# jason2714/de-i2i-gan

Measured on AMD Instinct MI355X. Metric: paired 256x256 images/sec (G+D train step), higher is better.
Workload: dtype bf16

## Files before the change

### de-i2i-gan_amd/_lib.py

```python
import ctypes
import os
from ctypes import POINTER, Structure, c_char_p, c_double, c_float, c_int, c_int64, c_size_t, c_uint64, c_void_p

_HERE = os.path.dirname(os.path.abspath(__file__))
LIB_PATH = os.path.join(_HERE, "lib", "libdei2i_hip.so")

BF16, F32 = 0, 1
ACT_NONE, ACT_RELU, ACT_LRELU = 0, 1, 2
PAD_ZERO, PAD_REFLECT = 0, 1
DIFFAUG_COLOR, DIFFAUG_TRANSLATION, DIFFAUG_CUTOUT, DIFFAUG_MAX_RUNS = 1, 2, 4, 16
PROF_GATHER_GEMM, PROF_WGRAD, PROF_HALO_CONV, PROF_HALO_FOLD = 0, 1, 2, 3


class ConvDesc(Structure):
    _fields_ = [("dtype", c_int), ("N", c_int), ("H", c_int), ("W", c_int), ("Cin", c_int), ("Cout", c_int),
                ("CinS", c_int), ("CoutS", c_int), ("kh", c_int), ("kw", c_int), ("stride", c_int), ("pad", c_int),
                ("pad_mode", c_int), ("up", c_int)]


class ProDesc(Structure):
    _fields_ = [("A", c_void_p), ("B", c_void_p), ("n_stride", c_int), ("slope", c_float), ("ring", c_void_p)]


class EpiNormDesc(Structure):
# ... 66 lines not shown
    "dei2i_compose_bwd": (c_int, [c_int, c_int, c_int, c_int, c_int, _P, _P, _P, _P, _P, _P, _P]),
    "dei2i_nan_guard": (c_int, [c_int, c_size_t, _P, _P, _P]),
    "dei2i_bce_logits_fwd": (c_int, [c_size_t, _P, _P, c_float, _P, _P]),
    "dei2i_bce_logits_bwd": (c_int, [c_size_t, _P, _P, c_float, _P, _P, _P]),
    "dei2i_l1_fwd": (c_int, [c_size_t, _P, _P, _P, _P]),
    "dei2i_l1_bwd": (c_int, [c_size_t, _P, _P, _P, _P, _P, _P]),
    "dei2i_noise_fwd": (c_int, [c_int, c_size_t, c_int, _P, _P, _P, _P, _P]),
    "dei2i_noise_bwd": (c_int, [c_int, c_size_t, c_int, _P, _P, _P, _P, c_int, _P]),
    "dei2i_spectral_scratch_floats": (c_size_t, [c_int, c_int]),
    "dei2i_spectral_fwd": (c_int, [c_int, c_int, _P, _P, _P, c_int, _P, _P, _P, _P, _P, _P]),
    "dei2i_spectral_bwd": (c_int, [c_int, c_int, _P, _P, _P, _P, _P, _P, _P, c_int, _P]),
    "dei2i_fold_bn_weight": (c_int, [c_int, c_int, _P, _P, _P, _P, _P, c_float, _P, _P, _P]),
    "dei2i_label_gb_packed_elems": (c_size_t, [c_int, c_int]),
    "dei2i_label_gb_pack": (c_int, [_P, c_int, c_int, _P]),
    "dei2i_label_gb_fwd": (c_int, [_P, c_int, c_int, c_int, c_int, _P, _P]),
    "dei2i_label_gb_dgrad": (c_int, [_P, c_int, c_int, c_int, c_int, _P, _P]),
    "dei2i_label_gb_wgrad": (c_int, [_P, c_int, c_int, c_int, c_int, _P, _P]),
    "dei2i_adam_step": (c_int, [_P, c_int, c_int64, c_float, c_float, c_float, c_float, c_float, c_float, c_float, c_float, _P]),
    "dei2i_sgd_rmsprop_step": (c_int, [_P, c_int, c_int64, c_int, c_float, c_float, c_float, c_float, _P]),
    "dei2i_adam_step_l2": (c_int, [_P, c_int, c_int64, c_float, c_float, c_float, c_float, c_float, c_float, c_float, c_float, _P]),
    "dei2i_adam_step_dev": (c_int, [_P, c_int, c_int64, _P, _P, c_int, c_float, c_float, c_float, c_float, _P]),
    "dei2i_adam_step_l2_dev": (c_int, [_P, c_int, c_int64, _P, _P, c_int, c_float, c_float, c_float, c_float, c_float, _P]),
    "dei2i_index_advance": (c_int, [_P, _P]),
    "dei2i_ema_lerp": (c_int, [_P, c_int, c_int64, c_float, _P]),
    "dei2i_diffaug_partial_floats": (c_size_t, [c_int]),
    "dei2i_diffaug": (c_int, [c_int, c_int, c_int, c_int, c_int, c_int, c_int, c_int, _P, _P, _P, _P, _P]),
    "dei2i_diffaug_draw": (c_int, [c_uint64, _P, c_int, c_uint64, c_int, c_int, c_int, c_int, _P, _P]),
    "dei2i_prof_enable": (c_int, [c_int, c_int]),
    "dei2i_prof_collect": (c_int, [c_int, POINTER(c_int64), POINTER(c_double), POINTER(c_double)]),
    "dei2i_prof_collect_timed": (c_int, [c_int, POINTER(c_int64), POINTER(c_double)]),
    "dei2i_conv2d_fused_supported": (c_int, [_CD, c_int]),
    "dei2i_conv2d_stats_chunks": (c_int, [_CD]),
    "dei2i_conv2d_fwd_fused": (c_int, [_CD, _P, _P, _P, c_int, _P, _PD, _P, _P]),
    "dei2i_conv2d_wgrad_pro_supported": (c_int, [_CD]),
    "dei2i_conv2d_wgrad_oihw_pro": (c_int, [_CD, _P, _P, _P, c_size_t, _P, c_int, _PD, _P]),
    "dei2i_ring_pixels": (c_size_t, [c_int, c_int]),
    "dei2i_conv2d_ring_supported": (c_int, [_CD]),
    "dei2i_conv2d_dgrad_norm_supported": (c_int, [_CD]),
    "dei2i_conv2d_dgrad_norm_chunks": (c_int, [_CD]),
    "dei2i_conv2d_dgrad_input_norm": (c_int, [_CD, _P, _P, _P, _ED, _P]),
    "dei2i_avgpool2_fwd": (c_int, [c_int, c_int, c_int, c_int, c_int, _P, _P, _P]),
    "dei2i_avgpool2_bwd": (c_int, [c_int, c_int, c_int, c_int, c_int, _P, _P, _P]),
    "dei2i_spade_bwd_border": (c_int, [c_int, c_int, c_int, c_int, c_int, c_int, _P, _P, _P, _P, _P, c_float, _P, _P]),
    "dei2i_conv2d_fwd_ring": (c_int, [_CD, _P, _P, _P, _P, c_int, _P, _P, _P]),
    "dei2i_affine_act_img_fwd": (c_int, [c_int, c_int, c_int, c_int, _P, _P, _P, c_float, _P, _P]),
    "dei2i_spade_prep": (c_int, [c_int, c_int, c_int, c_int, c_int, c_int, _P, _P, c_int, c_float, _P, _P, _P, _P, _P, _P, _P]),
# ... 43 lines not shown
```

### de-i2i-gan_amd/csrc/adam.hip

```cpp
#include <hip/hip_runtime.h>

#include "../../include/dei2i_hip.h"
#include "launch.h"

namespace dei2i {

template <bool COUPLED, bool DEV>
__global__ __launch_bounds__(256) void adam_kernel(const dei2i_adam_rec* __restrict__ table, float lr, float beta1,
                                                   float beta2, float eps, float bias_c1, float bias_c2_sqrt,
                                                   float grad_scale, float keep, float wd, const float* __restrict__ hyper,
                                                   const int* __restrict__ index, int rows) {
  const dei2i_adam_rec rec = table[blockIdx.y];
  if (DEV) {
    const int r = *index;
    if (r < 0 || r >= rows) return;
    lr = hyper[4 * r];
    bias_c1 = hyper[4 * r + 1];
    bias_c2_sqrt = hyper[4 * r + 2];
    if (!COUPLED) keep = hyper[4 * r + 3];
  }
  const float step_size = lr / bias_c1;
  const float inv_c2 = 1.f / bias_c2_sqrt;
  const int64_t n = rec.n;
  const int64_t n4 = ((reinterpret_cast<uintptr_t>(rec.p) | reinterpret_cast<uintptr_t>(rec.g) |
                       reinterpret_cast<uintptr_t>(rec.m) | reinterpret_cast<uintptr_t>(rec.v)) & 15) == 0 ? n / 4 : 0;
  const int64_t stride = (int64_t)gridDim.x * blockDim.x;
  for (int64_t i = (int64_t)blockIdx.x * blockDim.x + threadIdx.x; i < n4; i += stride) {
    float4 p = reinterpret_cast<float4*>(rec.p)[i];
    const float4 g = reinterpret_cast<const float4*>(rec.g)[i];
    float4 m = reinterpret_cast<float4*>(rec.m)[i];
    float4 v = reinterpret_cast<float4*>(rec.v)[i];
    float* pp = &p.x; const float* gp = &g.x; float* mp = &m.x; float* vp = &v.x;
#pragma unroll
    for (int e = 0; e < 4; ++e) {
      const float gv = COUPLED ? gp[e] * grad_scale + wd * pp[e] : gp[e] * grad_scale;
      mp[e] = mp[e] + (1.f - beta1) * (gv - mp[e]);
      vp[e] = beta2 * vp[e] + (1.f - beta2) * gv * gv;
      const float denom = sqrtf(vp[e]) * inv_c2 + eps;
      pp[e] = pp[e] * keep - step_size * (mp[e] / denom);
    }
    reinterpret_cast<float4*>(rec.p)[i] = p;
    reinterpret_cast<float4*>(rec.m)[i] = m;
    reinterpret_cast<float4*>(rec.v)[i] = v;
  }
  for (int64_t i = n4 * 4 + (int64_t)blockIdx.x * blockDim.x + threadIdx.x; i < n; i += stride) {
    const float gv = COUPLED ? rec.g[i] * grad_scale + wd * rec.p[i] : rec.g[i] * grad_scale;
    const float m = rec.m[i] + (1.f - beta1) * (gv - rec.m[i]);
    const float v = beta2 * rec.v[i] + (1.f - beta2) * gv * gv;
    rec.m[i] = m;
    rec.v[i] = v;
    rec.p[i] = rec.p[i] * keep - step_size * (m / (sqrtf(v) * inv_c2 + eps));
  }
}

__global__ __launch_bounds__(256) void sgd_rmsprop_kernel(const dei2i_adam_rec* __restrict__ table, int kind, float lr, float alpha,
                                                          float eps, float grad_scale) {
  const dei2i_adam_rec rec = table[blockIdx.y];
  const int64_t n = rec.n, stride = (int64_t)gridDim.x * blockDim.x;
  for (int64_t i = (int64_t)blockIdx.x * blockDim.x + threadIdx.x; i < n; i += stride) {
    const float gv = rec.g[i] * grad_scale;
    if (kind == 0) {
      rec.p[i] -= lr * gv;
    } else {
      const float sq = alpha * rec.m[i] + (1.f - alpha) * gv * gv;
      rec.m[i] = sq;
      rec.p[i] -= lr * (gv / (sqrtf(sq) + eps));
    }
  }
}

__global__ __launch_bounds__(256) void ema_lerp_kernel(const dei2i_adam_rec* __restrict__ table, float w) {
  const dei2i_adam_rec rec = table[blockIdx.y];
  const int64_t n = rec.n, stride = (int64_t)gridDim.x * blockDim.x;
  const bool hi = fabsf(w) >= 0.5f;
  for (int64_t i = (int64_t)blockIdx.x * blockDim.x + threadIdx.x; i < n; i += stride) {
// ... 48 lines not shown
  if (bx < 1) bx = 1;
  if (bx > 512) bx = 512;
  if (coupled)
    hipLaunchKernelGGL((adam_kernel<true, true>), dim3((unsigned)bx, (unsigned)count), dim3(256), 0, (hipStream_t)s, table_dev, 0.f,
                       beta1, beta2, eps, 1.f, 1.f, grad_scale, 1.f, weight_decay, hyper_dev, index_dev, rows);
  else
    hipLaunchKernelGGL((adam_kernel<false, true>), dim3((unsigned)bx, (unsigned)count), dim3(256), 0, (hipStream_t)s, table_dev, 0.f,
                       beta1, beta2, eps, 1.f, 1.f, grad_scale, 1.f, 0.f, hyper_dev, index_dev, rows);
  return (int)hipGetLastError();
}

extern "C" int dei2i_adam_step_dev(const dei2i_adam_rec* table_dev, int count, int64_t max_n, const float* hyper_dev,
                                   const int* index_dev, int rows, float beta1, float beta2, float eps, float grad_scale,
                                   dei2i_stream s) {
  return adam_dev_launch(false, table_dev, count, max_n, hyper_dev, index_dev, rows, beta1, beta2, eps, grad_scale, 0.f, s);
}

extern "C" int dei2i_adam_step_l2_dev(const dei2i_adam_rec* table_dev, int count, int64_t max_n, const float* hyper_dev,
                                      const int* index_dev, int rows, float beta1, float beta2, float eps, float grad_scale,
                                      float weight_decay, dei2i_stream s) {
  return adam_dev_launch(true, table_dev, count, max_n, hyper_dev, index_dev, rows, beta1, beta2, eps, grad_scale, weight_decay, s);
}

__global__ void index_advance_kernel(int* index) { *index += 1; }

extern "C" int dei2i_index_advance(int* index_dev, dei2i_stream s) {
  if (!index_dev) return DEI2I_ERR_BAD_ARG;
  hipLaunchKernelGGL(index_advance_kernel, dim3(1), dim3(1), 0, (hipStream_t)s, index_dev);
  return (int)hipGetLastError();
}

extern "C" int dei2i_ema_lerp(const dei2i_adam_rec* table_dev, int count, int64_t max_n, float weight, dei2i_stream s) {
  if (!table_dev || count <= 0 || max_n <= 0) return DEI2I_ERR_BAD_ARG;
  int64_t bx = (max_n + 255) / 256;
  if (bx < 1) bx = 1;
  if (bx > 1024) bx = 1024;
  hipLaunchKernelGGL(ema_lerp_kernel, dim3((unsigned)bx, (unsigned)count), dim3(256), 0, (hipStream_t)s, table_dev, weight);
  return (int)hipGetLastError();
}
```

### de-i2i-gan_amd/csrc/conv_api.hip

```cpp
#include <hip/hip_runtime.h>

#include "../../include/dei2i_hip.h"
#include "launch.h"

namespace dei2i {

static ConvShape to_shape(const dei2i_conv* c) {
  ConvShape s;
  s.N = c->N; s.H = c->H; s.W = c->W; s.Cin = c->Cin; s.Cout = c->Cout;
  s.kh = c->kh; s.kw = c->kw; s.stride = c->stride; s.pad = c->pad; s.pad_mode = c->pad_mode; s.up = c->up;
  return s;
}

static bool valid_conv(const dei2i_conv* c) {
  if (!c) return false;
  const int vec = c->dtype == DT_BF16 ? 8 : 4;
  if (c->dtype != DT_BF16 && c->dtype != DT_F32) return false;
  if (c->N <= 0 || c->H <= 0 || c->W <= 0 || c->Cin <= 0 || c->Cout <= 0) return false;
  if (c->CinS < c->Cin || c->CoutS < c->Cout || c->CinS % vec || c->CoutS % vec) return false;
  if (c->kh <= 0 || c->kw <= 0 || c->stride <= 0 || c->pad < 0 || c->up < 0 || c->up > 1) return false;
  if (c->kh < c->stride || c->kw < c->stride) return false;
  if (c->pad_mode == PAD_REFLECT && (c->pad >= (c->H << c->up) || c->pad >= (c->W << c->up))) return false;
  if (((c->H << c->up) + 2 * c->pad) < c->kh || ((c->W << c->up) + 2 * c->pad) < c->kw) return false;
  return true;
}

template <typename T>
__global__ void pack_fwd_kernel(const float* __restrict__ w, T* __restrict__ dst, int Cout, int Cin, int CinS, int kh, int kw) {
  const size_t total = (size_t)Cout * kh * kw * CinS;
  for (size_t i = (size_t)blockIdx.x * blockDim.x + threadIdx.x; i < total; i += (size_t)gridDim.x * blockDim.x) {
    const long long si = packed_fwd_src((long long)i, Cin, CinS, kh * kw);
    Elem<T>::store(dst + i, si >= 0 ? w[si] : 0.f);
  }
}

template <typename T>
__global__ void pack_dgrad_kernel(const float* __restrict__ w, T* __restrict__ dst, int Cout, int Cin, int CoutS, int kh,
                                  int kw, int s, int ay, int ax, int th, int tw) {
  const size_t total = (size_t)Cin * th * tw * CoutS;
  for (size_t i = (size_t)blockIdx.x * blockDim.x + threadIdx.x; i < total; i += (size_t)gridDim.x * blockDim.x) {
    const long long si = packed_dgrad_src((long long)i, Cout, Cin, CoutS, kh, kw, s, ay, ax, th, tw);
    Elem<T>::store(dst + i, si >= 0 ? w[si] : 0.f);
  }
}

struct PackAll {
  long long fwd_total;
  long long cls_begin[17];
  int ay[16], ax[16], th[16], tw[16];
  int ncls;
};
template <typename T>
__global__ void pack_all_kernel(const float* __restrict__ w, T* __restrict__ fwd, T* __restrict__ dgrad, const PackAll pa, int Cout,
                                int Cin, int CinS, int CoutS, int kh, int kw, int s) {
  const long long total = pa.fwd_total + pa.cls_begin[pa.ncls];
  for (long long i = (long long)blockIdx.x * blockDim.x + threadIdx.x; i < total; i += (long long)gridDim.x * blockDim.x) {
    if (i < pa.fwd_total) {
      const long long si = packed_fwd_src(i, Cin, CinS, kh * kw);
      Elem<T>::store(fwd + i, si >= 0 ? w[si] : 0.f);
    } else {
      const long long j = i - pa.fwd_total;
      int k = 0;
      while (k + 1 < pa.ncls && j >= pa.cls_begin[k + 1]) ++k;
      const long long si = packed_dgrad_src(j - pa.cls_begin[k], Cout, Cin, CoutS, kh, kw, s, pa.ay[k], pa.ax[k], pa.th[k], pa.tw[k]);
      Elem<T>::store(dgrad + j, si >= 0 ? w[si] : 0.f);
    }
  }
}

constexpr int PT_CO = 16, PT_CI = 32, PT_MAXTAPS = 16, PT_ROW = PT_CI + 1;
template <typename T>
__global__ __launch_bounds__(256) void pack_tiled_kernel(const float* __restrict__ w, T* __restrict__ fwd, T* __restrict__ dgrad,
                                                         const PackAll pa, int Cout, int Cin, int CinS, int CoutS, int kh, int kw, int s) {
  constexpr int VEC = Elem<T>::VEC;
  extern __shared__ float tile[];
  const int taps = kh * kw;
  const int ci0 = blockIdx.x * PT_CI, co0 = blockIdx.y * PT_CO;
  const int run = PT_CI * taps;
  {
    const int r0 = threadIdx.x, r1 = threadIdx.x + 256;
    const int cil0 = r0 / taps, t0 = r0 - cil0 * taps, cil1 = r1 / taps, t1 = r1 - cil1 * taps;
    const bool in0 = r0 < run && ci0 + cil0 < Cin, in1 = r1 < run && ci0 + cil1 < Cin;
    float v0[PT_CO], v1[PT_CO];
#pragma unroll
    for (int col = 0; col < PT_CO; ++col) {
      const float* wr = w + ((size_t)(co0 + col) * Cin + ci0) * taps;
      const bool row = co0 + col < Cout;
      v0[col] = (row && in0) ? wr[r0] : 0.f;
      v1[col] = (row && in1) ? wr[r1] : 0.f;
    }
#pragma unroll
    for (int col = 0; col < PT_CO; ++col) {
      if (r0 < run) tile[(col * taps + t0) * PT_ROW + cil0] = v0[col];
      if (r1 < run) tile[(col * taps + t1) * PT_ROW + cil1] = v1[col];
    }
  }
  __syncthreads();
  constexpr int FCH = PT_CI / VEC;
  for (int i = threadIdx.x; i < PT_CO * taps * FCH; i += 256) {
    const int ch = i % FCH, r = i / FCH;
    const int col = r / taps, t = r - col * taps;
    const int co = co0 + col, ci = ci0 + ch * VEC;
    if (co >= Cout || ci >= CinS) continue;
    float v[VEC];
#pragma unroll
    for (int e = 0; e < VEC; ++e) v[e] = tile[r * PT_ROW + ch * VEC + e];
    *reinterpret_cast<u32x4*>(fwd + ((size_t)co * taps + t) * CinS + ci) = Elem<T>::pack(v);
  }
  constexpr int DCH = PT_CO / VEC;
  for (int k = 0; k < pa.ncls; ++k) {
    const int th = pa.th[k], tw = pa.tw[k], nt = th * tw;
    T* dst = dgrad + pa.cls_begin[k];
    for (int i = threadIdx.x; i < PT_CI * nt * DCH; i += 256) {
      const int ch = i % DCH, r = i / DCH;
      const int t = r % nt, cil = r / nt;
      const int ci = ci0 + cil, co = co0 + ch * VEC;
      if (ci >= Cin || co >= CoutS) continue;
      const int jy = t / tw, jx = t - jy * tw;
      const int tap = (pa.ay[k] + s * jy) * kw + (pa.ax[k] + s * jx);
      float v[VEC];
#pragma unroll
      for (int e = 0; e < VEC; ++e) v[e] = tile[((ch * VEC + e) * taps + tap) * PT_ROW + cil];
      *reinterpret_cast<u32x4*>(dst + ((size_t)ci * nt + t) * CoutS + co) = Elem<T>::pack(v);
    }
  }
}

template <typename T>
__global__ void fold_pad_kernel(const T* __restrict__ ext, const T* __restrict__ addend, T* __restrict__ dx, int N, int H,
                                int W, int C, int pad, int reflect, int up) {
  constexpr int VEC = Elem<T>::VEC;
  const int Hl = H << up, Wl = W << up;
  const int off = reflect ? pad : 0;
  const int OH = Hl + 2 * off, OW = Wl + 2 * off;
  const int cv = C / VEC;
  const size_t total = (size_t)N * H * W * cv;
  for (size_t i = (size_t)blockIdx.x * blockDim.x + threadIdx.x; i < total; i += (size_t)gridDim.x * blockDim.x) {
    const int c = (int)(i % cv) * VEC;
    size_t r = i / cv;
    const int w = (int)(r % W); r /= W;
    const int h = (int)(r % H);
    const int n = (int)(r / H);
    float acc[VEC];
#pragma unroll
    for (int e = 0; e < VEC; ++e) acc[e] = 0.f;
    if (addend != nullptr) {
      float t[VEC];
      Elem<T>::unpack(*reinterpret_cast<const u32x4*>(addend + i * VEC), t);
// ... 82 lines not shown
  return (int)hipGetLastError();
}

int dei2i_pack_weight_dgrad(const dei2i_conv* c, const float* w, void* packed, dei2i_stream s) {
  if (!valid_conv(c) || !w || !packed) return DEI2I_ERR_BAD_ARG;
  hipStream_t st = (hipStream_t)s;
  const size_t esz = c->dtype == DT_BF16 ? 2 : 4;
  for_each_dgrad_class(c->Cin, c->CoutS, c->kh, c->kw, c->stride, [&](const DgradClass& k) {
    if (k.count == 0) return;
    const unsigned grid = grid_for((size_t)k.count, 256);
    void* dst = (char*)packed + (size_t)k.off * esz;
    by_dtype(c->dtype, [&](auto t) {
      using T = decltype(t);
      hipLaunchKernelGGL(pack_dgrad_kernel<T>, dim3(grid), dim3(256), 0, st, w, (T*)dst, c->Cout, c->Cin, c->CoutS, c->kh, c->kw,
                         c->stride, k.ay, k.ax, k.th, k.tw);
    });
  });
  return (int)hipGetLastError();
}

int dei2i_pack_weight_both(const dei2i_conv* c, const float* w, void* packed_fwd, void* packed_dgrad, dei2i_stream s) {
  if (!valid_conv(c) || !w || !packed_fwd || !packed_dgrad || c->stride > 4) return DEI2I_ERR_BAD_ARG;
  PackAll pa;
  pa.fwd_total = (long long)dei2i_packed_fwd_elems(c);
  pa.ncls = 0;
  const long long off = for_each_dgrad_class(c->Cin, c->CoutS, c->kh, c->kw, c->stride, [&](const DgradClass& k) {
    if (k.count == 0) return;
    pa.ay[pa.ncls] = k.ay; pa.ax[pa.ncls] = k.ax; pa.th[pa.ncls] = k.th; pa.tw[pa.ncls] = k.tw;
    pa.cls_begin[pa.ncls++] = k.off;
  });
  pa.cls_begin[pa.ncls] = off;
  for (int k = pa.ncls + 1; k < 17; ++k) pa.cls_begin[k] = off;
  if (c->kh * c->kw <= PT_MAXTAPS && (long long)c->Cout * c->Cin * c->kh * c->kw >= (1 << 16) && c->CoutS % 8 == 0) {
    const dim3 tg((c->CinS + PT_CI - 1) / PT_CI, (c->CoutS + PT_CO - 1) / PT_CO);
    const size_t plds = (size_t)PT_CO * c->kh * c->kw * PT_ROW * sizeof(float);
    hipError_t e = hipSuccess;
    by_dtype(c->dtype, [&](auto t) {
      using T = decltype(t);
      e = ensure_dyn_lds(reinterpret_cast<const void*>(pack_tiled_kernel<T>), plds);
      if (e != hipSuccess) return;
      hipLaunchKernelGGL(pack_tiled_kernel<T>, tg, dim3(256), plds, (hipStream_t)s, w, (T*)packed_fwd, (T*)packed_dgrad, pa, c->Cout,
                         c->Cin, c->CinS, c->CoutS, c->kh, c->kw, c->stride);
      e = hipGetLastError();
    });
    return (int)e;
  }
  const unsigned grid = grid_for((size_t)(pa.fwd_total + off), 256);
  by_dtype(c->dtype, [&](auto t) {
    using T = decltype(t);
    hipLaunchKernelGGL(pack_all_kernel<T>, dim3(grid), dim3(256), 0, (hipStream_t)s, w, (T*)packed_fwd, (T*)packed_dgrad, pa, c->Cout,
                       c->Cin, c->CinS, c->CoutS, c->kh, c->kw, c->stride);
  });
  return (int)hipGetLastError();
}

void dei2i_conv2d_out_shape(const dei2i_conv* c, int* Ho, int* Wo) {
  *Ho = conv_out_dim(c->H << c->up, c->kh, c->stride, c->pad);
  *Wo = conv_out_dim(c->W << c->up, c->kw, c->stride, c->pad);
}

void dei2i_conv2d_dgrad_shape(const dei2i_conv* c, int* OH, int* OW) {
  ConvShape s = to_shape(c);
  *OH = dgrad_out_h(s);
  *OW = dgrad_out_w(s);
}

size_t dei2i_conv2d_workspace_bytes(const dei2i_conv* c) {
  int Ho, Wo, OH, OW;
  dei2i_conv2d_out_shape(c, &Ho, &Wo);
  dei2i_conv2d_dgrad_shape(c, &OH, &OW);
  const size_t f = (size_t)c->N * Ho * Wo * c->CoutS, d = (size_t)c->N * OH * OW * c->CinS;
  const size_t one = (f > d ? f : d) * sizeof(float);
  const size_t many = one * 16, cap = one > ((size_t)64 << 20) ? one : ((size_t)64 << 20);
  return many < cap ? many : cap;
}

// ... 231 lines not shown
```

### de-i2i-gan_amd/ops.py

```python
from __future__ import annotations

import ctypes
import weakref
from ctypes import byref, c_int, c_void_p
from dataclasses import dataclass
from typing import Optional

import torch

from . import _lib as L

ACT = {"none": L.ACT_NONE, None: L.ACT_NONE, "relu": L.ACT_RELU, "leaky_relu": L.ACT_LRELU}


@dataclass(frozen=True)
class Precision:
    name: str
    code: int
    dtype: torch.dtype
    vec: int

    def pad(self, c: int) -> int:
        return (c + self.vec - 1) // self.vec * self.vec

# ... 275 lines not shown
    cin: int
    cout: int
    k: int
    stride: int = 1
    pad: int = 0
    reflect: bool = False
    up: bool = False


_descs = {}


def _desc(prec: Precision, g: ConvGeom, n: int, h: int, w: int, cins: int, couts: int) -> L.ConvDesc:
    key = (prec.code, g, n, h, w, cins, couts)
    d = _descs.get(key)
    if d is None:
        if len(_descs) > 4096:
            _descs.clear()
        d = _descs[key] = L.ConvDesc(prec.code, n, h, w, g.cin, g.cout, cins, couts, g.k, g.k, g.stride, g.pad,
                                     L.PAD_REFLECT if g.reflect else L.PAD_ZERO, 1 if g.up else 0)
    return d


class PackedWeights:

    def __init__(self):
        self._key = None
        self.fwd = None
        self.dgrad = None
        self.fp8 = None
        self._packed_on = None

    def _mark_packed(self):
        ev = self._packed_on[1] if self._packed_on is not None else torch.cuda.Event()
        ev.record()
        self._packed_on = (_stream_id(), ev, capture_serial)

    def _await_pack(self):
        if self._packed_on is not None and self._packed_on[0] != _stream_id():
            if self._packed_on[2] != capture_serial and torch.cuda.is_current_stream_capturing():
                return
            torch.cuda.current_stream().wait_event(self._packed_on[1])

    @staticmethod
    def _stamp(t: torch.Tensor):
        return (t.data_ptr(), t._version, getattr(t, "_dei2i_epoch", 0))

    def get(self, weight: torch.Tensor, sources, prec: Precision, geom: ConvGeom, cins: int, couts: int, need_dgrad: bool,
            need_fwd: bool = True, per_call: bool = False):
        key = ((), prec.code, cins, couts, self._stamp(weight)) if per_call else \
            (tuple(self._stamp(s) for s in sources), prec.code, cins, couts, None)
        if key == self._key and (self.fwd is not None or not need_fwd) and (self.dgrad is not None or not need_dgrad):
            self._await_pack()
            return self.fwd, self.dgrad
        lib = _lib_for(weight)
        if key != self._key:
            self._key, self.fwd, self.dgrad, self.fp8 = key, None, None, None
        d = _desc(prec, geom, 1, max(geom.k, 4), max(geom.k, 4), cins, couts)
        w = weight.detach()
        if w.dtype != torch.float32 or not w.is_contiguous():
            w = w.float().contiguous()
        self._await_pack()
        packed = False
        if need_fwd and need_dgrad and self.fwd is None and self.dgrad is None:
            self.fwd = torch.empty(lib.dei2i_packed_fwd_elems(byref(d)), dtype=prec.dtype, device=weight.device)
            self.dgrad = torch.empty(lib.dei2i_packed_dgrad_elems(byref(d)), dtype=prec.dtype, device=weight.device)
            L.check(lib.dei2i_pack_weight_both(byref(d), _p(w), _p(self.fwd), _p(self.dgrad), _stream()), "pack_weight_both")
            packed = True
        if need_fwd and self.fwd is None:
            self.fwd = torch.empty(lib.dei2i_packed_fwd_elems(byref(d)), dtype=prec.dtype, device=weight.device)
            L.check(lib.dei2i_pack_weight_fwd(byref(d), _p(w), _p(self.fwd), _stream()), "pack_weight_fwd")
            packed = True
        if need_dgrad and self.dgrad is None:
            self.dgrad = torch.empty(lib.dei2i_packed_dgrad_elems(byref(d)), dtype=prec.dtype, device=weight.device)
            L.check(lib.dei2i_pack_weight_dgrad(byref(d), _p(w), _p(self.dgrad), _stream()), "pack_weight_dgrad")
            packed = True
        if packed:
            self._mark_packed()
        return self.fwd, self.dgrad

    def get_fp8(self, weight: torch.Tensor, sources, prec: Precision, geom: ConvGeom, cins: int, couts: int):
        key = (tuple(self._stamp(s) for s in sources), prec.code, cins, couts, None)
        if key != self._key:
            self._key, self.fwd, self.dgrad, self.fp8 = key, None, None, None
        if self.fp8 is None:
            lib = _lib_for(weight)
            d = _desc(prec, geom, 1, 8, 32, cins, couts)
            w = weight.detach()
            if w.dtype != torch.float32 or not w.is_contiguous():
                w = w.float().contiguous()
            amax = torch.linalg.vector_norm(w, ord=float("inf")).reshape(1)
            wq = torch.empty(geom.cout * geom.k * geom.k * cins, dtype=torch.uint8, device=weight.device)
            dequant = torch.empty(1, dtype=torch.float32, device=weight.device)
            L.check(lib.dei2i_pack_weight_fwd_fp8(byref(d), _p(w), _p(amax), FP8_ACT_SCALE, _p(wq), _p(dequant), _stream()),
                    "pack_weight_fwd_fp8")
            self.fp8 = (wq, dequant)
        return self.fp8


def _stats_of(t, n, hw, c):
    st = getattr(t, "_dei2i_stats", None)
# ... 1449 lines not shown
```

### de-i2i-gan_amd/optim.py

```python
import ctypes
import math

import numpy as np
import torch

from . import _lib as L
from . import ops


class FusedAdam(torch.optim.Optimizer):
    def __init__(self, params, lr=1e-3, betas=(0.9, 0.999), eps=1e-8, grad_scale=1.0, weight_decay=0.0, decoupled=True):
        if lr < 0.0 or eps < 0.0 or weight_decay < 0.0 or not (0.0 <= betas[0] < 1.0) or not (0.0 <= betas[1] < 1.0):
            raise ValueError("invalid Adam hyper-parameter")
        super().__init__(params, dict(lr=lr, betas=betas, eps=eps, weight_decay=weight_decay))
        self.grad_scale = float(grad_scale)
        self.decoupled = bool(decoupled)

    @torch.no_grad()
    def step(self, closure=None):
        loss = None
        if closure is not None:
            with torch.enable_grad():
                loss = closure()
        if torch.cuda.is_current_stream_capturing():
            self._step_captured()
            return loss
        for group in self.param_groups:
            by_step = {}
            for p in group["params"]:
                if p.grad is None:
                    continue
                ops._require_gpu(p, "FusedAdam")
                if p.dtype != torch.float32 or p.grad.dtype != torch.float32:
                    raise TypeError("FusedAdam expects fp32 parameters and gradients")
                st = self.state[p]
                if len(st) == 0:
                    st["step"] = 0
                    st["exp_avg"] = torch.zeros_like(p, memory_format=torch.contiguous_format)
                    st["exp_avg_sq"] = torch.zeros_like(p, memory_format=torch.contiguous_format)
                st["step"] += 1
                by_step.setdefault(st["step"], []).append(p)
            b1, b2 = group["betas"]
            wd = float(group.get("weight_decay", 0.0))
            for t, plist in by_step.items():
                self._launch(plist, t, float(group["lr"]), b1, b2, group["eps"], wd, coupled=wd > 0.0 and not self.decoupled)
        return loss

    def _launch(self, plist, t, lr, b1, b2, eps, weight_decay=0.0, coupled=False):
        dev = plist[0].device
        lib = ops._lib_for(plist[0])
        n = len(plist)
        rows = []
        max_n = 0
        for p in plist:
            g = p.grad if p.grad.is_contiguous() else p.grad.contiguous()
            if not p.is_contiguous():
                raise RuntimeError("FusedAdam: non-contiguous parameter")
            st = self.state[p]
            rows.append((p.data_ptr(), g.data_ptr(), st["exp_avg"].data_ptr(), st["exp_avg_sq"].data_ptr(), p.numel()))
            max_n = max(max_n, p.numel())
            p._dei2i_keep = g
        cache = self.__dict__.setdefault("_table_cache", {})
        key = (dev, n, rows[0][0])
        hit = cache.get(key)
        if hit is not None and hit[0] == rows:
            table_dev = hit[1]
        else:
            table = torch.empty((n, 5), dtype=torch.int64, pin_memory=True)
            table.copy_(torch.tensor(rows, dtype=torch.int64))
# ... 230 lines not shown
```

### include/dei2i_hip.h

```cpp
#ifndef DEI2I_HIP_H
#define DEI2I_HIP_H

#include <stddef.h>
#include <stdint.h>

#ifdef __cplusplus
extern "C" {
#endif

typedef void* dei2i_stream;

#define DEI2I_BF16 0
#define DEI2I_F32 1
#define DEI2I_ACT_NONE 0
#define DEI2I_ACT_RELU 1
#define DEI2I_ACT_LRELU 2
#define DEI2I_PAD_ZERO 0
#define DEI2I_PAD_REFLECT 1

#define DEI2I_ERR_BAD_ARG (-2)
#define DEI2I_ERR_WORKSPACE (-3)

typedef struct dei2i_conv {
  int dtype;
// ... 96 lines not shown
                    dei2i_stream s);
int dei2i_noise_bwd(int dtype, size_t rows, int C, const void* dy, const float* noise, float* partials, float* dweight,
                    int accumulate, dei2i_stream s);

typedef struct dei2i_adam_rec {
  float* p;
  const float* g;
  float* m;
  float* v;
  int64_t n;
} dei2i_adam_rec;
int dei2i_adam_step(const dei2i_adam_rec* table_dev, int count, int64_t max_n, float lr, float beta1, float beta2,
                    float eps, float bias_c1, float bias_c2_sqrt, float grad_scale, float decoupled_decay, dei2i_stream s);
int dei2i_sgd_rmsprop_step(const dei2i_adam_rec* table_dev, int count, int64_t max_n, int kind, float lr, float alpha, float eps,
                           float grad_scale, dei2i_stream s);

int dei2i_adam_step_l2(const dei2i_adam_rec* table_dev, int count, int64_t max_n, float lr, float beta1, float beta2, float eps,
                       float bias_c1, float bias_c2_sqrt, float grad_scale, float weight_decay, dei2i_stream s);
int dei2i_adam_step_dev(const dei2i_adam_rec* table_dev, int count, int64_t max_n, const float* hyper_dev, const int* index_dev,
                        int rows, float beta1, float beta2, float eps, float grad_scale, dei2i_stream s);
int dei2i_adam_step_l2_dev(const dei2i_adam_rec* table_dev, int count, int64_t max_n, const float* hyper_dev, const int* index_dev,
                           int rows, float beta1, float beta2, float eps, float grad_scale, float weight_decay, dei2i_stream s);
int dei2i_index_advance(int* index_dev, dei2i_stream s);
int dei2i_ema_lerp(const dei2i_adam_rec* table_dev, int count, int64_t max_n, float weight, dei2i_stream s);

typedef struct dei2i_diffaug_rec {
  float a, b, k, beta;
  int ty, tx, top, left;
} dei2i_diffaug_rec;
size_t dei2i_diffaug_partial_floats(int N);
int dei2i_diffaug(int mode, int N, int C, int H, int W, int ch, int cw, int color, const float* src, const dei2i_diffaug_rec* tab,
                  float* partial, float* dst, dei2i_stream s);
#define DEI2I_DIFFAUG_COLOR 1
#define DEI2I_DIFFAUG_TRANSLATION 2
#define DEI2I_DIFFAUG_CUTOUT 4
#define DEI2I_DIFFAUG_MAX_RUNS 16
int dei2i_diffaug_draw(uint64_t seed, uint64_t* counter_dev, int runs, uint64_t run_flags, int N, int row0, int H, int W,
                       dei2i_diffaug_rec* tab, dei2i_stream s);

size_t dei2i_spectral_scratch_floats(int Cout, int K);
int dei2i_spectral_fwd(int Cout, int K, const float* W, float* u, float* v, int iterate, float* scratch, float* u_used,
                       float* v_used, float* scal, float* w_eff, dei2i_stream s);
int dei2i_spectral_bwd(int Cout, int K, const float* G, const float* w_eff, const float* u_used, const float* v_used,
                       const float* scal, float* scratch, float* dW, int accumulate, dei2i_stream s);

int dei2i_fold_bn_weight(int Cout, int K, const float* W, const float* bn_weight, const float* bn_bias, const float* running_mean,
// ... 86 lines not shown
```

Baseline: 472.5.

## Fuse Adam update with bf16 weight repacking for conv weights

Adds a tiled Adam kernel that updates each conv weight tile and, in the same pass, writes the bf16 forward and dgrad packed weight layouts through shared memory. The optimizer registers a sink on each parameter so the PackedWeights cache is marked fresh after the step. This removes the separate read-and-pack pass that would otherwise run before the next forward. It adds coupling between the optimizer and the conv pack cache, plus cache-invalidation bookkeeping that must stay consistent.

```diff
diff --git a/de-i2i-gan_amd/_lib.py b/de-i2i-gan_amd/_lib.py
--- a/de-i2i-gan_amd/_lib.py
+++ b/de-i2i-gan_amd/_lib.py
@@ -112,6 +112,10 @@
     "dei2i_adam_step_dev": (c_int, [_P, c_int, c_int64, _P, _P, c_int, c_float, c_float, c_float, c_float, _P]),
     "dei2i_adam_step_l2_dev": (c_int, [_P, c_int, c_int64, _P, _P, c_int, c_float, c_float, c_float, c_float, c_float, _P]),
     "dei2i_index_advance": (c_int, [_P, _P]),
+    "dei2i_adam_pack_rec_bytes": (c_size_t, []),
+    "dei2i_adam_pack_rec_fill": (c_int, [_CD, _P, _P, _P, _P, _P, _P, c_int, _P]),
+    "dei2i_adam_pack_step": (c_int, [_P, c_int, c_int, c_int, c_float, c_float, c_float, c_float, c_float, c_float, c_float, c_float,
+                                     _P, _P, c_int, _P]),
     "dei2i_ema_lerp": (c_int, [_P, c_int, c_int64, c_float, _P]),
     "dei2i_diffaug_partial_floats": (c_size_t, [c_int]),
     "dei2i_diffaug": (c_int, [c_int, c_int, c_int, c_int, c_int, c_int, c_int, c_int, _P, _P, _P, _P, _P]),
diff --git a/de-i2i-gan_amd/csrc/adam.hip b/de-i2i-gan_amd/csrc/adam.hip
--- a/de-i2i-gan_amd/csrc/adam.hip
+++ b/de-i2i-gan_amd/csrc/adam.hip
@@ -1,6 +1,7 @@
 #include <hip/hip_runtime.h>
 
 #include "../../include/dei2i_hip.h"
+#include "adam_pack.h"
 #include "launch.h"
 
 namespace dei2i {
@@ -11,14 +12,7 @@
                                                    float grad_scale, float keep, float wd, const float* __restrict__ hyper,
                                                    const int* __restrict__ index, int rows) {
   const dei2i_adam_rec rec = table[blockIdx.y];
-  if (DEV) {
-    const int r = *index;
-    if (r < 0 || r >= rows) return;
-    lr = hyper[4 * r];
-    bias_c1 = hyper[4 * r + 1];
-    bias_c2_sqrt = hyper[4 * r + 2];
-    if (!COUPLED) keep = hyper[4 * r + 3];
-  }
+  if (!adam_hyper<COUPLED, DEV>(lr, bias_c1, bias_c2_sqrt, keep, hyper, index, rows)) return;
   const float step_size = lr / bias_c1;
   const float inv_c2 = 1.f / bias_c2_sqrt;
   const int64_t n = rec.n;
@@ -32,25 +26,96 @@
     float4 v = reinterpret_cast<float4*>(rec.v)[i];
     float* pp = &p.x; const float* gp = &g.x; float* mp = &m.x; float* vp = &v.x;
 #pragma unroll
-    for (int e = 0; e < 4; ++e) {
-      const float gv = COUPLED ? gp[e] * grad_scale + wd * pp[e] : gp[e] * grad_scale;
-      mp[e] = mp[e] + (1.f - beta1) * (gv - mp[e]);
-      vp[e] = beta2 * vp[e] + (1.f - beta2) * gv * gv;
-      const float denom = sqrtf(vp[e]) * inv_c2 + eps;
-      pp[e] = pp[e] * keep - step_size * (mp[e] / denom);
-    }
+    for (int e = 0; e < 4; ++e) adam_update<COUPLED, false>(pp[e], gp[e], mp[e], vp[e], beta1, beta2, eps, step_size, inv_c2, grad_scale, keep, wd);
     reinterpret_cast<float4*>(rec.p)[i] = p;
     reinterpret_cast<float4*>(rec.m)[i] = m;
     reinterpret_cast<float4*>(rec.v)[i] = v;
   }
   for (int64_t i = n4 * 4 + (int64_t)blockIdx.x * blockDim.x + threadIdx.x; i < n; i += stride) {
-    const float gv = COUPLED ? rec.g[i] * grad_scale + wd * rec.p[i] : rec.g[i] * grad_scale;
-    const float m = rec.m[i] + (1.f - beta1) * (gv - rec.m[i]);
-    const float v = beta2 * rec.v[i] + (1.f - beta2) * gv * gv;
+    float p = rec.p[i], m = rec.m[i], v = rec.v[i];
+    adam_update<COUPLED, true>(p, rec.g[i], m, v, beta1, beta2, eps, step_size, inv_c2, grad_scale, keep, wd);
     rec.m[i] = m;
     rec.v[i] = v;
-    rec.p[i] = rec.p[i] * keep - step_size * (m / (sqrtf(v) * inv_c2 + eps));
-  }
+    rec.p[i] = p;
+  }
+}
+
+template <bool COUPLED, int W>
+__device__ __forceinline__ void adam_tile_rows(const AdamPackRec& rec, float* tile, bool aligned, int co0, int ci0, int taps, float beta1,
+                                               float beta2, float eps, float step_size, float inv_c2, float grad_scale, float keep,
+                                               float wd) {
+  const int runv = PT_CI * taps / W;
+  const int valid = rec.Cin - ci0 > 0 ? (rec.Cin - ci0 < PT_CI ? rec.Cin - ci0 : PT_CI) * taps : 0;
+  const size_t row_stride = (size_t)rec.Cin * taps;
+  const size_t body = ((size_t)rec.Cout * row_stride) & ~(size_t)3;
+  for (int i = threadIdx.x; i < PT_CO * runv; i += 256) {
+    const int col = i / runv, r = (i - col * runv) * W;
+    alignas(16) float p[W];
+#pragma unroll
+    for (int e = 0; e < W; ++e) p[e] = 0.f;
+    if (co0 + col < rec.Cout && r < valid) {
+      const size_t at = (size_t)(co0 + col) * row_stride + (size_t)ci0 * taps + r;
+      alignas(16) float g[W], m[W], v[W];
+      if constexpr (W == 4) {
+        *reinterpret_cast<float4*>(p) = *reinterpret_cast<const float4*>(rec.p + at);
+        *reinterpret_cast<float4*>(g) = *reinterpret_cast<const float4*>(rec.g + at);
+        *reinterpret_cast<float4*>(m) = *reinterpret_cast<const float4*>(rec.m + at);
+        *reinterpret_cast<float4*>(v) = *reinterpret_cast<const float4*>(rec.v + at);
+      } else {
+        p[0] = rec.p[at]; g[0] = rec.g[at]; m[0] = rec.m[at]; v[0] = rec.v[at];
+      }
+      if (W == 1 && (!aligned || at >= body)) {
+        adam_update<COUPLED, true>(p[0], g[0], m[0], v[0], beta1, beta2, eps, step_size, inv_c2, grad_scale, keep, wd);
+      } else {
+#pragma unroll
+        for (int e = 0; e < W; ++e)
+          adam_update<COUPLED, false>(p[e], g[e], m[e], v[e], beta1, beta2, eps, step_size, inv_c2, grad_scale, keep, wd);
+      }
+      if constexpr (W == 4) {
+        *reinterpret_cast<float4*>(rec.p + at) = *reinterpret_cast<const float4*>(p);
+        *reinterpret_cast<float4*>(rec.m + at) = *reinterpret_cast<const float4*>(m);
+        *reinterpret_cast<float4*>(rec.v + at) = *reinterpret_cast<const float4*>(v);
+      } else {
+        rec.p[at] = p[0]; rec.m[at] = m[0]; rec.v[at] = v[0];
+      }
+    }
+    int cil = r / taps, t = r - cil * taps;
+#pragma unroll
+    for (int e = 0; e < W; ++e) {
+      tile[(col * taps + t) * PT_ROW + cil] = p[e];
+      if (++t == taps) { t = 0; ++cil; }
+    }
+  }
+}
+
+template <bool COUPLED, bool DEV>
+__global__ __launch_bounds__(256) void adam_pack_tiled_kernel(const AdamPackRec* __restrict__ table, int count, float lr, float beta1,
+                                                              float beta2, float eps, float bias_c1, float bias_c2_sqrt,
+                                                              float grad_scale, float keep, float wd,
+                                                              const float* __restrict__ hyper, const int* __restrict__ index,
+                                                              int rows) {
+  extern __shared__ float tile[];
+  if (!adam_hyper<COUPLED, DEV>(lr, bias_c1, bias_c2_sqrt, keep, hyper, index, rows)) return;
+  const float step_size = lr / bias_c1;
+  const float inv_c2 = 1.f / bias_c2_sqrt;
+  int lo = 0, hi = count - 1;
+  while (lo < hi) {
+    const int mid = (lo + hi + 1) >> 1;
+    if (table[mid].tile_begin <= (int)blockIdx.x) lo = mid; else hi = mid - 1;
+  }
+  const AdamPackRec& rec = table[lo];
+  const int tl = (int)blockIdx.x - rec.tile_begin;
+  if (tl < 0 || tl >= rec.tile_count) return;
+  const int ty = tl / rec.tiles_x, tx = tl - ty * rec.tiles_x;
+  const int co0 = ty * PT_CO, ci0 = tx * PT_CI, taps = rec.kh * rec.kw;
+  const bool aligned = ((reinterpret_cast<uintptr_t>(rec.p) | reinterpret_cast<uintptr_t>(rec.g) | reinterpret_cast<uintptr_t>(rec.m) |
+                         reinterpret_cast<uintptr_t>(rec.v)) & 15) == 0;
+  if (aligned && (((size_t)rec.Cin * taps) & 3) == 0)
+    adam_tile_rows<COUPLED, 4>(rec, tile, aligned, co0, ci0, taps, beta1, beta2, eps, step_size, inv_c2, grad_scale, keep, wd);
+  else
+    adam_tile_rows<COUPLED, 1>(rec, tile, aligned, co0, ci0, taps, beta1, beta2, eps, step_size, inv_c2, grad_scale, keep, wd);
+  __syncthreads();
+  pack_tile_store<bf16_t>(tile, rec.fwd, rec.dgrad, rec.pa, co0, ci0, rec.Cout, rec.Cin, rec.CinS, rec.CoutS, taps, rec.kw, rec.s);
 }
 
 __global__ __launch_bounds__(256) void sgd_rmsprop_kernel(const dei2i_adam_rec* __restrict__ table, int kind, float lr, float alpha,
@@ -145,6 +210,31 @@
   return adam_dev_launch(true, table_dev, count, max_n, hyper_dev, index_dev, rows, beta1, beta2, eps, grad_scale, weight_decay, s);
 }
 
+extern "C" int dei2i_adam_pack_step(const void* recs_dev, int count, int total_tiles, int coupled, float lr, float beta1, float beta2,
+                                    float eps, float bias_c1, float bias_c2_sqrt, float grad_scale, float decay, const float* hyper_dev,
+                                    const int* index_dev, int rows, dei2i_stream s) {
+  if (!recs_dev || count <= 0 || total_tiles <= 0) return DEI2I_ERR_BAD_ARG;
+  const bool dev = hyper_dev != nullptr;
+  if (dev && (!index_dev || rows <= 0)) return DEI2I_ERR_BAD_ARG;
+  const AdamPackRec* table = static_cast<const AdamPackRec*>(recs_dev);
+  const dim3 grid((unsigned)total_tiles), block(256);
+  const size_t lds = (size_t)PT_CO * PT_MAXTAPS * PT_ROW * sizeof(float);
+  const hipStream_t st = (hipStream_t)s;
+  if (coupled && dev)
+    hipLaunchKernelGGL((adam_pack_tiled_kernel<true, true>), grid, block, lds, st, table, count, 0.f, beta1, beta2, eps, 1.f, 1.f,
+                       grad_scale, 1.f, decay, hyper_dev, index_dev, rows);
+  else if (coupled)
+    hipLaunchKernelGGL((adam_pack_tiled_kernel<true, false>), grid, block, lds, st, table, count, lr, beta1, beta2, eps, bias_c1,
+                       bias_c2_sqrt, grad_scale, 1.f, decay, nullptr, nullptr, 0);
+  else if (dev)
+    hipLaunchKernelGGL((adam_pack_tiled_kernel<false, true>), grid, block, lds, st, table, count, 0.f, beta1, beta2, eps, 1.f, 1.f,
+                       grad_scale, 1.f, 0.f, hyper_dev, index_dev, rows);
+  else
+    hipLaunchKernelGGL((adam_pack_tiled_kernel<false, false>), grid, block, lds, st, table, count, lr, beta1, beta2, eps, bias_c1,
+                       bias_c2_sqrt, grad_scale, 1.f - lr * decay, 0.f, nullptr, nullptr, 0);
+  return (int)hipGetLastError();
+}
+
 __global__ void index_advance_kernel(int* index) { *index += 1; }
 
 extern "C" int dei2i_index_advance(int* index_dev, dei2i_stream s) {
diff --git a/de-i2i-gan_amd/csrc/adam_pack.h b/de-i2i-gan_amd/csrc/adam_pack.h
--- /dev/null
+++ b/de-i2i-gan_amd/csrc/adam_pack.h
@@ -0,0 +1,114 @@
+#pragma once
+#include "common.h"
+#include "geom.h"
+
+namespace dei2i {
+
+struct PackAll {
+  long long fwd_total;
+  long long cls_begin[17];
+  int ay[16], ax[16], th[16], tw[16];
+  int ncls;
+};
+
+inline long long fill_pack_all(PackAll& pa, long long fwd_total, int Cin, int CoutS, int kh, int kw, int stride) {
+  pa.fwd_total = fwd_total;
+  pa.ncls = 0;
+  const long long off = for_each_dgrad_class(Cin, CoutS, kh, kw, stride, [&](const DgradClass& k) {
+    if (k.count == 0) return;
+    pa.ay[pa.ncls] = k.ay; pa.ax[pa.ncls] = k.ax; pa.th[pa.ncls] = k.th; pa.tw[pa.ncls] = k.tw;
+    pa.cls_begin[pa.ncls++] = k.off;
+  });
+  for (int k = pa.ncls; k < 16; ++k) pa.ay[k] = pa.ax[k] = pa.th[k] = pa.tw[k] = 0;
+  for (int k = pa.ncls; k < 17; ++k) pa.cls_begin[k] = off;
+  return off;
+}
+
+constexpr int PT_CO = 16, PT_CI = 32, PT_MAXTAPS = 16, PT_ROW = PT_CI + 1;
+
+struct AdamPackRec {
+  float* p;
+  const float* g;
+  float* m;
+  float* v;
+  uint16_t* fwd;
+  uint16_t* dgrad;
+  int Cout, Cin, CinS, CoutS, kh, kw, s;
+  int tiles_x, tile_begin, tile_count;
+  PackAll pa;
+};
+
+#if defined(__HIPCC__)
+
+template <typename T>
+DEI2I_D void pack_tile_store(const float* tile, T* __restrict__ fwd, T* __restrict__ dgrad, const PackAll& pa, int co0, int ci0,
+                             int Cout, int Cin, int CinS, int CoutS, int taps, int kw, int s) {
+  constexpr int VEC = Elem<T>::VEC;
+  constexpr int FCH = PT_CI / VEC;
+  for (int i = threadIdx.x; i < PT_CO * taps * FCH; i += 256) {
+    const int ch = i % FCH, r = i / FCH;
+    const int col = r / taps, t = r - col * taps;
+    const int co = co0 + col, ci = ci0 + ch * VEC;
+    if (co >= Cout || ci >= CinS) continue;
+    float v[VEC];
+#pragma unroll
+    for (int e = 0; e < VEC; ++e) v[e] = tile[r * PT_ROW + ch * VEC + e];
+    *reinterpret_cast<u32x4*>(fwd + ((size_t)co * taps + t) * CinS + ci) = Elem<T>::pack(v);
+  }
+  constexpr int DCH = PT_CO / VEC;
+  for (int k = 0; k < pa.ncls; ++k) {
+    const int th = pa.th[k], tw = pa.tw[k], nt = th * tw;
+    T* dst = dgrad + pa.cls_begin[k];
+    for (int i = threadIdx.x; i < PT_CI * nt * DCH; i += 256) {
+      const int ch = i % DCH, r = i / DCH;
+      const int t = r % nt, cil = r / nt;
+      const int ci = ci0 + cil, co = co0 + ch * VEC;
+      if (ci >= Cin || co >= CoutS) continue;
+      const int jy = t / tw, jx = t - jy * tw;
+      const int tap = (pa.ay[k] + s * jy) * kw + (pa.ax[k] + s * jx);
+      float v[VEC];
+#pragma unroll
+      for (int e = 0; e < VEC; ++e) v[e] = tile[((ch * VEC + e) * taps + tap) * PT_ROW + cil];
+      *reinterpret_cast<u32x4*>(dst + ((size_t)ci * nt + t) * CoutS + co) = Elem<T>::pack(v);
+    }
+  }
+}
+
+template <bool COUPLED, bool DEV>
+DEI2I_D bool adam_hyper(float& lr, float& bias_c1, float& bias_c2_sqrt, float& keep, const float* __restrict__ hyper,
+                        const int* __restrict__ index, int rows) {
+  if (DEV) {
+    const int r = *index;
+    if (r < 0 || r >= rows) return false;
+    lr = hyper[4 * r];
+    bias_c1 = hyper[4 * r + 1];
+    bias_c2_sqrt = hyper[4 * r + 2];
+    if (!COUPLED) keep = hyper[4 * r + 3];
+  }
+  return true;
+}
+
+template <bool COUPLED, bool TAIL>
+DEI2I_D void adam_update(float& p, float g, float& m, float& v, float beta1, float beta2, float eps, float step_size, float inv_c2,
+                         float grad_scale, float keep, float wd) {
+#pragma clang fp contract(off)
+  float gv, d;
+  if (COUPLED) {
+    gv = TAIL ? __builtin_fmaf(wd, p, g * grad_scale) : __builtin_fmaf(grad_scale, g, wd * p);
+    d = gv - m;
+  } else {
+    gv = g * grad_scale;
+    d = __builtin_fmaf(grad_scale, g, -m);
+  }
+  m = __builtin_fmaf(1.f - beta1, d, m);
+  const float c = (1.f - beta2) * gv;
+  if (TAIL) v = beta2 * v + gv * c;
+  else if (COUPLED) v = __builtin_fmaf(beta2, v, gv * c);
+  else v = __builtin_fmaf(gv, c, beta2 * v);
+  const float q = m / __builtin_fmaf(inv_c2, sqrtf(v), eps);
+  p = TAIL ? keep * p - step_size * q : __builtin_fmaf(keep, p, -(step_size * q));
+}
+
+#endif
+
+}
diff --git a/de-i2i-gan_amd/csrc/conv_api.hip b/de-i2i-gan_amd/csrc/conv_api.hip
--- a/de-i2i-gan_amd/csrc/conv_api.hip
+++ b/de-i2i-gan_amd/csrc/conv_api.hip
@@ -1,6 +1,8 @@
 #include <hip/hip_runtime.h>
+#include <string.h>
 
 #include "../../include/dei2i_hip.h"
+#include "adam_pack.h"
 #include "launch.h"
 
 namespace dei2i {
@@ -44,12 +46,6 @@
   }
 }
 
-struct PackAll {
-  long long fwd_total;
-  long long cls_begin[17];
-  int ay[16], ax[16], th[16], tw[16];
-  int ncls;
-};
 template <typename T>
 __global__ void pack_all_kernel(const float* __restrict__ w, T* __restrict__ fwd, T* __restrict__ dgrad, const PackAll pa, int Cout,
                                 int Cin, int CinS, int CoutS, int kh, int kw, int s) {
@@ -68,11 +64,9 @@
   }
 }
 
-constexpr int PT_CO = 16, PT_CI = 32, PT_MAXTAPS = 16, PT_ROW = PT_CI + 1;
 template <typename T>
 __global__ __launch_bounds__(256) void pack_tiled_kernel(const float* __restrict__ w, T* __restrict__ fwd, T* __restrict__ dgrad,
                                                          const PackAll pa, int Cout, int Cin, int CinS, int CoutS, int kh, int kw, int s) {
-  constexpr int VEC = Elem<T>::VEC;
   extern __shared__ float tile[];
   const int taps = kh * kw;
   const int ci0 = blockIdx.x * PT_CI, co0 = blockIdx.y * PT_CO;
@@ -96,34 +90,7 @@
     }
   }
   __syncthreads();
-  constexpr int FCH = PT_CI / VEC;
-  for (int i = threadIdx.x; i < PT_CO * taps * FCH; i += 256) {
-    const int ch = i % FCH, r = i / FCH;
-    const int col = r / taps, t = r - col * taps;
-    const int co = co0 + col, ci = ci0 + ch * VEC;
-    if (co >= Cout || ci >= CinS) continue;
-    float v[VEC];
-#pragma unroll
-    for (int e = 0; e < VEC; ++e) v[e] = tile[r * PT_ROW + ch * VEC + e];
-    *reinterpret_cast<u32x4*>(fwd + ((size_t)co * taps + t) * CinS + ci) = Elem<T>::pack(v);
-  }
-  constexpr int DCH = PT_CO / VEC;
-  for (int k = 0; k < pa.ncls; ++k) {
-    const int th = pa.th[k], tw = pa.tw[k], nt = th * tw;
-    T* dst = dgrad + pa.cls_begin[k];
-    for (int i = threadIdx.x; i < PT_CI * nt * DCH; i += 256) {
-      const int ch = i % DCH, r = i / DCH;
-      const int t = r % nt, cil = r / nt;
-      const int ci = ci0 + cil, co = co0 + ch * VEC;
-      if (ci >= Cin || co >= CoutS) continue;
-      const int jy = t / tw, jx = t - jy * tw;
-      const int tap = (pa.ay[k] + s * jy) * kw + (pa.ax[k] + s * jx);
-      float v[VEC];
-#pragma unroll
-      for (int e = 0; e < VEC; ++e) v[e] = tile[((ch * VEC + e) * taps + tap) * PT_ROW + cil];
-      *reinterpret_cast<u32x4*>(dst + ((size_t)ci * nt + t) * CoutS + co) = Elem<T>::pack(v);
-    }
-  }
+  pack_tile_store<T>(tile, fwd, dgrad, pa, co0, ci0, Cout, Cin, CinS, CoutS, taps, kw, s);
 }
 
 template <typename T>
@@ -252,15 +219,7 @@
 int dei2i_pack_weight_both(const dei2i_conv* c, const float* w, void* packed_fwd, void* packed_dgrad, dei2i_stream s) {
   if (!valid_conv(c) || !w || !packed_fwd || !packed_dgrad || c->stride > 4) return DEI2I_ERR_BAD_ARG;
   PackAll pa;
-  pa.fwd_total = (long long)dei2i_packed_fwd_elems(c);
-  pa.ncls = 0;
-  const long long off = for_each_dgrad_class(c->Cin, c->CoutS, c->kh, c->kw, c->stride, [&](const DgradClass& k) {
-    if (k.count == 0) return;
-    pa.ay[pa.ncls] = k.ay; pa.ax[pa.ncls] = k.ax; pa.th[pa.ncls] = k.th; pa.tw[pa.ncls] = k.tw;
-    pa.cls_begin[pa.ncls++] = k.off;
-  });
-  pa.cls_begin[pa.ncls] = off;
-  for (int k = pa.ncls + 1; k < 17; ++k) pa.cls_begin[k] = off;
+  const long long off = fill_pack_all(pa, (long long)dei2i_packed_fwd_elems(c), c->Cin, c->CoutS, c->kh, c->kw, c->stride);
   if (c->kh * c->kw <= PT_MAXTAPS && (long long)c->Cout * c->Cin * c->kh * c->kw >= (1 << 16) && c->CoutS % 8 == 0) {
     const dim3 tg((c->CinS + PT_CI - 1) / PT_CI, (c->CoutS + PT_CO - 1) / PT_CO);
     const size_t plds = (size_t)PT_CO * c->kh * c->kw * PT_ROW * sizeof(float);
@@ -282,6 +241,27 @@
                        c->Cin, c->CinS, c->CoutS, c->kh, c->kw, c->stride);
   });
   return (int)hipGetLastError();
+}
+
+size_t dei2i_adam_pack_rec_bytes(void) { return sizeof(AdamPackRec); }
+
+int dei2i_adam_pack_rec_fill(const dei2i_conv* c, float* p, const float* g, float* m, float* v, void* packed_fwd, void* packed_dgrad,
+                             int tile_begin, void* rec_host) {
+  if (!valid_conv(c) || c->dtype != DT_BF16 || c->stride > 4 || c->kh * c->kw > PT_MAXTAPS || !p || !g || !m || !v || !packed_fwd ||
+      !packed_dgrad || tile_begin < 0 || !rec_host)
+    return DEI2I_ERR_BAD_ARG;
+  AdamPackRec r;
+  r.p = p; r.g = g; r.m = m; r.v = v;
+  r.fwd = (uint16_t*)packed_fwd; r.dgrad = (uint16_t*)packed_dgrad;
+  r.Cout = c->Cout; r.Cin = c->Cin; r.CinS = c->CinS; r.CoutS = c->CoutS; r.kh = c->kh; r.kw = c->kw; r.s = c->stride;
+  r.tiles_x = (c->CinS + PT_CI - 1) / PT_CI;
+  const long long tiles = (long long)r.tiles_x * ((c->CoutS + PT_CO - 1) / PT_CO);
+  if (tiles > 0x7fffffffLL - tile_begin) return DEI2I_ERR_BAD_ARG;
+  r.tile_begin = tile_begin;
+  r.tile_count = (int)tiles;
+  fill_pack_all(r.pa, (long long)dei2i_packed_fwd_elems(c), c->Cin, c->CoutS, c->kh, c->kw, c->stride);
+  memcpy(rec_host, &r, sizeof(r));
+  return r.tile_count;
 }
 
 void dei2i_conv2d_out_shape(const dei2i_conv* c, int* Ho, int* Wo) {
diff --git a/de-i2i-gan_amd/ops.py b/de-i2i-gan_amd/ops.py
--- a/de-i2i-gan_amd/ops.py
+++ b/de-i2i-gan_amd/ops.py
@@ -321,7 +321,29 @@
     return d
 
 
+adam_packs = True
+
+
+class _PackSink:
+    __slots__ = ("cache", "key", "fwd", "dgrad", "desc")
+
+    def __init__(self, cache, key, fwd, dgrad, desc):
+        self.cache, self.key, self.fwd, self.dgrad, self.desc = weakref.ref(cache), key, fwd, dgrad, desc
+
+    def __reduce__(self):
+        return (type(None), ())
+
+    def live(self, p):
+        cache = self.cache()
+        if (cache is None or cache._key is not self.key or cache.fwd is not self.fwd or cache.dgrad is not self.dgrad
+                or self.key[0][0] != PackedWeights._stamp(p)):
+            return None
+        return cache
+
+
 class PackedWeights:
+
+    launches = {"plain": 0, "other": 0}
 
     def __init__(self):
         self._key = None
@@ -329,11 +351,20 @@
         self.dgrad = None
         self.fp8 = None
         self._packed_on = None
+        self._event = None
 
     def _mark_packed(self):
-        ev = self._packed_on[1] if self._packed_on is not None else torch.cuda.Event()
+        ev = self._event
+        if ev is None:
+            ev = self._event = torch.cuda.Event()
         ev.record()
         self._packed_on = (_stream_id(), ev, capture_serial)
+
+    def adam_wrote(self, sink, p, event):
+        key = self._key
+        self._key = sink.key = ((self._stamp(p),),) + key[1:]
+        self.fp8 = None
+        self._packed_on = (_stream_id(), event, capture_serial)
 
     def _await_pack(self):
         if self._packed_on is not None and self._packed_on[0] != _stream_id():
@@ -376,6 +407,13 @@
             packed = True
         if packed:
             self._mark_packed()
+            src = sources[0] if not per_call and len(sources) == 1 else None
+            plain = (src is not None and isinstance(src, torch.nn.Parameter) and w.data_ptr() == src.data_ptr()
+                     and src.shape == weight.shape and prec is BF16 and geom.k * geom.k <= 16 and geom.stride <= 4)
+            self.launches["plain" if plain else "other"] += 1
+            if (plain and adam_packs and self.fwd is not None and self.dgrad is not None
+                    and not torch.cuda.is_current_stream_capturing()):
+                src._dei2i_sink = _PackSink(self, self._key, self.fwd, self.dgrad, d)
         return self.fwd, self.dgrad
 
     def get_fp8(self, weight: torch.Tensor, sources, prec: Precision, geom: ConvGeom, cins: int, couts: int):
diff --git a/de-i2i-gan_amd/optim.py b/de-i2i-gan_amd/optim.py
--- a/de-i2i-gan_amd/optim.py
+++ b/de-i2i-gan_amd/optim.py
@@ -39,12 +39,59 @@
                     st["exp_avg"] = torch.zeros_like(p, memory_format=torch.contiguous_format)
                     st["exp_avg_sq"] = torch.zeros_like(p, memory_format=torch.contiguous_format)
                 st["step"] += 1
-                by_step.setdefault(st["step"], []).append(p)
+                sink = getattr(p, "_dei2i_sink", None)
+                if sink is not None and not (ops.adam_packs and p.is_contiguous() and sink.live(p) is not None):
+                    sink = p._dei2i_sink = None
+                by_step.setdefault((st["step"], sink is not None), []).append(p)
             b1, b2 = group["betas"]
             wd = float(group.get("weight_decay", 0.0))
-            for t, plist in by_step.items():
-                self._launch(plist, t, float(group["lr"]), b1, b2, group["eps"], wd, coupled=wd > 0.0 and not self.decoupled)
+            for (t, tiled), plist in by_step.items():
+                launch = self._launch_tiled if tiled else self._launch
+                launch(plist, t, float(group["lr"]), b1, b2, group["eps"], wd, coupled=wd > 0.0 and not self.decoupled)
         return loss
+
+    def _launch_tiled(self, plist, t, lr, b1, b2, eps, weight_decay=0.0, coupled=False):
+        dev = plist[0].device
+        lib = ops._lib_for(plist[0])
+        rows = []
+        for p in plist:
+            g = p.grad if p.grad.is_contiguous() else p.grad.contiguous()
+            st, sink = self.state[p], p._dei2i_sink
+            rows.append((p.data_ptr(), g.data_ptr(), st["exp_avg"].data_ptr(), st["exp_avg_sq"].data_ptr(), sink.fwd.data_ptr(),
+                         sink.dgrad.data_ptr(), id(sink.desc)))
+            p._dei2i_keep = g
+        cache = self.__dict__.setdefault("_tile_table_cache", {})
+        key = (dev, len(plist), rows[0][0])
+        hit = cache.get(key)
+        if hit is not None and hit[0] == rows:
+            table_dev, tiles = hit[1], hit[2]
+        else:
+            nbytes = lib.dei2i_adam_pack_rec_bytes()
+            table = torch.empty((len(plist), nbytes), dtype=torch.uint8, pin_memory=True)
+            tiles = 0
+            for i, (p, r) in enumerate(zip(plist, rows)):
+                count = lib.dei2i_adam_pack_rec_fill(ctypes.byref(p._dei2i_sink.desc), *(ctypes.c_void_p(a) for a in r[:6]), tiles,
+                                                     ctypes.c_void_p(table.data_ptr() + i * nbytes))
+                if count <= 0:
+                    L.check(count or -2, "adam_pack_rec_fill")
+                tiles += count
+            table_dev = table.to(dev, non_blocking=True)
+            cache[key] = (rows, table_dev, tiles, [p._dei2i_sink.desc for p in plist])
+        L.check(lib.dei2i_adam_pack_step(ctypes.c_void_p(table_dev.data_ptr()), len(plist), tiles, 1 if coupled else 0, lr, b1, b2, eps,
+                                         1.0 - b1 ** t, math.sqrt(1.0 - b2 ** t), self.grad_scale, weight_decay, None, None, 0,
+                                         ops._stream()), "adam_pack_step")
+        sid = ops._stream_id()
+        event = self.__dict__.setdefault("_pack_events", {}).get(sid)
+        if event is None:
+            event = self._pack_events[sid] = torch.cuda.Event()
+        event.record()
+        for p in plist:
+            p._dei2i_epoch = getattr(p, "_dei2i_epoch", 0) + 1
+            p._dei2i_keep = None
+            sink = p._dei2i_sink
+            owner = sink.cache()
+            if owner is not None:
+                owner.adam_wrote(sink, p, event)
 
     def _launch(self, plist, t, lr, b1, b2, eps, weight_decay=0.0, coupled=False):
         dev = plist[0].device
diff --git a/include/dei2i_hip.h b/include/dei2i_hip.h
--- a/include/dei2i_hip.h
+++ b/include/dei2i_hip.h
@@ -142,6 +142,12 @@
 int dei2i_adam_step_l2_dev(const dei2i_adam_rec* table_dev, int count, int64_t max_n, const float* hyper_dev, const int* index_dev,
                            int rows, float beta1, float beta2, float eps, float grad_scale, float weight_decay, dei2i_stream s);
 int dei2i_index_advance(int* index_dev, dei2i_stream s);
+size_t dei2i_adam_pack_rec_bytes(void);
+int dei2i_adam_pack_rec_fill(const dei2i_conv* c, float* p, const float* g, float* m, float* v, void* packed_fwd, void* packed_dgrad,
+                             int tile_begin, void* rec_host);
+int dei2i_adam_pack_step(const void* recs_dev, int count, int total_tiles, int coupled, float lr, float beta1, float beta2,
+                         float eps, float bias_c1, float bias_c2_sqrt, float grad_scale, float decay, const float* hyper_dev,
+                         const int* index_dev, int rows, dei2i_stream s);
 int dei2i_ema_lerp(const dei2i_adam_rec* table_dev, int count, int64_t max_n, float weight, dei2i_stream s);
 
 typedef struct dei2i_diffaug_rec {
```

After: 476.1 (median of 6 runs). No clear change (+0.8%).
